# proroklab/graph-conv-memory

Hardware: AMD Instinct MI355X
Metric: belief-states/sec (BxT) DenseGCM fwd+bwd, graph_size=128 F=32 (higher is better)
Workload: dtype f32; 1 GPU; cfg2: DenseGCM + TemporalBackedge([1,2,4]), B=256/GPU, graph_size=128, obs=32, hidden=32, 2x DenseGraphConv+tanh, T=128; one bench step = one rollout through the per-step drop-in call surface `for t: mx, m = gcm(obs[t], m)` + backward; B_per_gpu=256, graph_size=128, obs=32, hidden=32, T=128, state=donated (DenseGCM(donate_state=True): hidden state advanced in place), parallelism=dp1 (batch-sharded, 1 flat-bucket all-reduce per backward)

## Files before the change

graph-conv-memory_amd/csrc/rows_cached_run.hip:

```cpp
#include <atomic>
#include <new>
#include <type_traits>

#include "fused_common.h"
#include "gcm_common.h"
#include "rows_common.h"
#include "rows_head.h"
#include "rows_lean.h"

namespace gcm_rows {

constexpr int RUN_CAP = GCM_ROWS_MAX_STEPS;
constexpr int RUN_WAVES = 8;
constexpr int RUN_PAIRS = RUN_CAP / 2 / RUN_WAVES;
constexpr int RUN_OCTS = RUN_CAP / 8 / RUN_WAVES;
constexpr int RUN_WSTAGE = 2 * 16 * 64 / (64 * RUN_WAVES);

struct RunTable {
  const float* obs[RUN_CAP];
  float* rec[RUN_CAP];
};

struct FreshArgs {
  HeadSrcs hs;
  float* packed;
  float* image;
  unsigned pad0, pad0_end, pad1, pad1_end;
};
struct NoFresh {};
constexpr int RUN_ADJ_TAB = 256 + 128;

#ifndef GCM_RUN_FRESH_STORES_LATE
#define GCM_RUN_FRESH_STORES_LATE 0
#endif

template <bool FRESH>
__global__ __launch_bounds__(64 * RUN_WAVES) void k_step_rows_cached_img4_lean_run(
    const float* __restrict__ image, float* __restrict__ nodes, float* __restrict__ cH, const float* __restrict__ params,
    int cur0_arg, int n, unsigned hops4, unsigned nhs, float* __restrict__ adj, int64_t* __restrict__ count,
    float* __restrict__ cA, float* __restrict__ cX, uint32_t* __restrict__ flags, unsigned o_v, unsigned o_hdr,
    unsigned o_coef, unsigned o_live, int rec, RunTable tab, std::conditional_t<FRESH, FreshArgs, NoFresh> fr) {
  constexpr int F = 32, H1 = 32, ROWS = 128 * 32;
  const int cur0 = FRESH ? 0 : cur0_arg;
  __shared__ __attribute__((aligned(16))) float sXH[2 * ROWS];
  __shared__ __attribute__((aligned(16))) float svw[RUN_WAVES * 128];
  __shared__ __attribute__((aligned(16))) f32x2 sW[2 * 16 * 32 * 2];
  __shared__ float sadj[FRESH ? RUN_ADJ_TAB : 1];
  const int lane = threadIdx.x & 63;
  const int wv = __builtin_amdgcn_readfirstlane((int)(threadIdx.x >> 6));
  const unsigned gb = blockIdx.x;
  const unsigned N = nhs & 0xffu;
  const int H2 = (int)((nhs >> 8) & 0xffu);
  const bool self = (nhs >> 16) & 1u;
  const unsigned g0 = gb * N;
  const int fl = lane & 31, hs = lane >> 5;
  float* sv = svw + 128 * wv + 64 * hs;
  const int ol = fl < H2 ? fl : H2 - 1;
  float* recd[RUN_OCTS];
#pragma unroll
  for (int j = 0; j < RUN_OCTS; ++j) {
    const int t = 8 * (wv + RUN_WAVES * j) + (lane >> 3);
    recd[j] = tab.rec[t < n ? t : n - 1];
  }
  float xo[RUN_PAIRS];
  float* recp[RUN_PAIRS];
#pragma unroll
  for (int j = 0; j < RUN_PAIRS; ++j) {
    const int t = 2 * (wv + RUN_WAVES * j) + hs;
    const int tc = t < n ? t : n - 1;
    xo[j] = tab.obs[tc][gb * F + fl];
    recp[j] = tab.rec[tc];
  }
  f32x2 wst[RUN_WSTAGE];
  f32x4 wq[2];
  float bias1, bias2;
  float v_img = 0.f, v_pack = 0.f;
  const size_t e_first = (size_t)gb + (size_t)gridDim.x * threadIdx.x, e_wave = (size_t)gb + (size_t)gridDim.x * (64 * wv);
  if constexpr (!FRESH) {
    const f32x2* i3 = reinterpret_cast<const f32x2*>(image + 2 * 4 * 64 * 64);
#pragma unroll
    for (int r = 0; r < RUN_WSTAGE; ++r) wst[r] = i3[(int)threadIdx.x + 64 * RUN_WAVES * r];
    const float* b1 = params + 2 * H1 * F;
    bias1 = b1[fl];
    bias2 = b1[H1 + 2 * H2 * H1 + ol];
  } else {
#pragma unroll
    for (int r = 0; r < 2; ++r) {
      const int q = (int)threadIdx.x + 64 * RUN_WAVES * r;
      const int m = q >> 8, h = (q >> 3) & 31;
      const float* w = m == 0 ? fr.hs.p[0] : m == 1 ? fr.hs.p[1] : m == 2 ? fr.hs.p[3] : fr.hs.p[4];
      wq[r] = f32x4{0.f, 0.f, 0.f, 0.f};
      if (m < 2 || h < H2) wq[r] = *reinterpret_cast<const f32x4*>(w + h * 32 + 4 * (q & 7));
    }
    bias1 = fr.hs.p[2][fl];
    bias2 = fr.hs.p[5][ol];
    if (e_wave < (size_t)IMG_LAYOUT_FLOATS && e_first < (size_t)IMG_LAYOUT_FLOATS) {
      const int e = (int)e_first;
      v_img = head_image_value(fr.hs, e >> 12, (e >> 6) & 63, e & 63, F, H1, H2);
    }
    if (e_wave < fr.hs.off[HEAD_MAX_SRCS] && e_first < fr.hs.off[HEAD_MAX_SRCS])
      v_pack = head_packed_value(fr.hs, (unsigned)e_first);
  }
  int hmax = 0, nh = 0;
#pragma unroll
  for (int i = 0; i < 4; ++i) {
    const int h = (int)((hops4 >> (8 * i)) & 0xffu);
    if (h != 0xff) {
      ++nh;
      if (h > hmax) hmax = h;
    }
  }
  {
    const int lo = cur0 - hmax > 0 ? cur0 - hmax : 0;
    const float* src = hs ? cH : nodes;
    for (int r = lo + wv; r < cur0; r += RUN_WAVES) sXH[hs * ROWS + r * 32 + fl] = src[(g0 + (unsigned)r) * 32 + fl];
  }
  if constexpr (!FRESH) {
#pragma unroll
    for (int r = 0; r < RUN_WSTAGE; ++r) {
      const int e = (int)threadIdx.x + 64 * RUN_WAVES * r;
      sW[image3_lds_pair(e)] = wst[r];
    }
  } else {
    float* sWf = reinterpret_cast<float*>(sW);
#pragma unroll
    for (int r = 0; r < 2; ++r) {
      const int q = (int)threadIdx.x + 64 * RUN_WAVES * r;
#pragma unroll
      for (int u = 0; u < 4; ++u) sWf[image3_lds_index(q >> 8, 4 * (q & 7) + u, (q >> 3) & 31)] = wq[r][u];
    }
    if (threadIdx.x < RUN_ADJ_TAB) {
      const int d = 128 - (int)threadIdx.x;
      bool hit = d == 0 && self;
#pragma unroll
      for (int i = 0; i < 4; ++i) hit = hit || (d > 0 && (int)((hops4 >> (8 * i)) & 0xffu) == d);
      sadj[threadIdx.x] = hit && threadIdx.x < 256 ? 1.f : 0.f;
    }
  }
#pragma unroll
  for (int j = 0; j < RUN_PAIRS; ++j) {
    const int t = 2 * (wv + RUN_WAVES * j) + hs;
    if (t < n) {
      sXH[(cur0 + t) * 32 + fl] = xo[j];
      const unsigned at = (g0 + (unsigned)(cur0 + t)) * F + fl;
      nodes[at] = xo[j];
      cX[at] = xo[j];
    }
  }
  __syncthreads();
  auto fresh_stores = [&]() {
    if constexpr (FRESH) {
      const f32x4 z = {0.f, 0.f, 0.f, 0.f};
      const int nq = (int)(N >> 2);
      f32x4* arow = reinterpret_cast<f32x4*>(adj + (size_t)g0 * N);
      for (int r = 2 * wv + hs; r < (int)N; r += 2 * RUN_WAVES) {
        if (fl < nq) {
          const float* at = sadj + (r < n ? 128 + 4 * fl - r : 256);
          arow[r * nq + fl] = f32x4{at[0], at[1], at[2], at[3]};
        }
      }
      f32x4* nrow = reinterpret_cast<f32x4*>(nodes + (size_t)g0 * F);
      for (int i = n * (F / 4) + (int)threadIdx.x; i < (int)N * (F / 4); i += 64 * RUN_WAVES) nrow[i] = z;
      if (gb == 0 && threadIdx.x < 64) {
        if (fr.pad0 + threadIdx.x < fr.pad0_end) nodes[fr.pad0 + threadIdx.x] = 0.f;
        if (fr.pad1 + threadIdx.x < fr.pad1_end) nodes[fr.pad1 + threadIdx.x] = 0.f;
      }
// ... 21 lines not shown
  for (int q = 0; q < 4; ++q) {
    const int idx = nh - 1 - q;
    has[q] = idx >= 0;
    back[q] = has[q] ? 32 * (int)((hops4 >> (8 * (idx & 3))) & 0xffu) : 0;
  }
  auto sources_all = [&](int cur, const float* rows, float (&va)[4]) {
    const float* at = rows + cur * 32 + fl;
#pragma unroll
    for (int q = 0; q < 4; ++q) {
      const float v = *(at - back[q]);
      va[q] = has[q] ? v : 0.f;
    }
  };
  f32x2 wa[16], wb[16];
  auto weights = [&](int layer) {
#pragma unroll
    for (int k = 0; k < 16; ++k) {
      const f32x4 q = *reinterpret_cast<const f32x4*>(sW + ((layer * 16 + k) * 32 + fl) * 2);
      wa[k] = f32x2{q[0], q[1]};
      wb[k] = f32x2{q[2], q[3]};
    }
  };
  auto matvec = [&]() { return lean_half_chain(wa, sv, 0) + lean_half_chain(wb, sv, 1); };
  weights(0);
  auto layer1 = [&](int cur, bool live, const float (&xa)[4]) {
    const unsigned rc = g0 + (unsigned)cur;
    const float xc = sXH[cur * 32 + fl];
    asm volatile("" ::: "memory");
    float agg1 = (xa[0] + xa[1]) + (xa[2] + xa[3]);
    agg1 = agg1 + (self ? xc : 0.f);
    *reinterpret_cast<f32x2*>(sv + 2 * fl) = f32x2{agg1, xc};
    asm volatile("" ::: "memory");
    const float p1 = bias1 + matvec();
    const float h1c = gcm_tanh(p1);
    asm volatile("" ::: "memory");
    if (live) {
      sXH[ROWS + cur * 32 + fl] = h1c;
      cA[rc * F + fl] = agg1;
      cH[rc * H1 + fl] = h1c;
    }
  };
#pragma unroll
  for (int j = 0; j < RUN_PAIRS; ++j) {
    const int t0 = 2 * (wv + RUN_WAVES * j);
    if (t0 >= n) break;
    const bool live = t0 + hs < n;
    const int cur = cur0 + (live ? t0 + hs : n - 1);
    float xa[4];
    if (cur0 + t0 < hmax) sources(cur, sXH, xa);
    else sources_all(cur, sXH, xa);
    layer1(cur, live, xa);
  }
  __syncthreads();
  weights(1);
  bool bad = false;
  auto layer2 = [&](int cur, bool live, float* saved, const float (&ha)[4]) {
    const float h1c = sXH[ROWS + cur * 32 + fl];
    asm volatile("" ::: "memory");
    float agg2 = (ha[0] + ha[1]) + (ha[2] + ha[3]);
    agg2 = agg2 + (self ? h1c : 0.f);
    *reinterpret_cast<f32x2*>(sv + 2 * fl) = f32x2{agg2, h1c};
    asm volatile("" ::: "memory");
    const float p2 = bias2 + matvec();
    const float v = gcm_tanh(p2);
    asm volatile("" ::: "memory");
    if (live && fl < H2) saved[gb * H2 + fl] = v;
    if (rec && live) {
      saved[o_v + gb * 2 * H1 + fl] = agg2;
      saved[o_v + gb * 2 * H1 + H1 + fl] = h1c;
    }
    bad = bad || (live && fl < H2 && !isfinite(v));
  };
#pragma unroll
  for (int j = 0; j < RUN_PAIRS; ++j) {
    const int t0 = 2 * (wv + RUN_WAVES * j);
    if (t0 >= n) break;
    const bool live = t0 + hs < n;
    const int cur = cur0 + (live ? t0 + hs : n - 1);
    float ha[4];
    if (cur0 + t0 < hmax) sources(cur, sXH + ROWS, ha);
    else sources_all(cur, sXH + ROWS, ha);
    layer2(cur, live, recp[j], ha);
  }
#pragma unroll
  for (int o = 0; o < RUN_OCTS; ++o) {
    const int t = 8 * (wv + RUN_WAVES * o) + (lane >> 3);
    if (t < n) {
      const int q = lane & 7;
      const int cur = cur0 + t;
      int k = 0;
#pragma unroll
      for (int i = 0; i < 4; ++i) k += (int)(((hops4 >> (8 * i)) & 0xffu) <= (unsigned)cur);
      const int j = q < k ? cur - (int)((hops4 >> (8 * ((k - 1 - q) & 3))) & 0xffu) : cur;
      const bool is_cur = q == k;
      if (!FRESH && (q < k || (is_cur && self))) adj[(size_t)(g0 + (unsigned)cur) * N + j] = 1.f;
      if (rec) {
        float* saved = recd[o];
        if (q <= k) {
          (reinterpret_cast<int*>(saved + o_live) + gb * N)[q] = j;
          (saved + o_coef + gb * N)[q] = (is_cur && !self) ? 0.f : 1.f;
        }
        if (q == 7) {
          int* hdr = reinterpret_cast<int*>(saved + o_hdr) + 4 * gb;
          hdr[0] = k + 1; hdr[1] = k; hdr[2] = cur; hdr[3] = 0;
        }
// ... 19 lines not shown
  int n = 0, cur0 = 0;
  float *nodes = nullptr, *adj = nullptr, *cH = nullptr, *cA = nullptr, *cX = nullptr;
  int64_t* count = nullptr;
  const float *params = nullptr, *image = nullptr;
  uint32_t* flags = nullptr;
  int B = 0, N = 0, H2 = 0, self = 0, rec = 0;
  unsigned hops4 = 0xffffffffu;
  RunTable tab;
  int cap = RUN_CAP;
  unsigned long long stat_cid = 0;
  int stat_nodes = 0, stat_merged = 0, stat_absorbed = 0;
  struct Head {
    hipGraphNode_t node = nullptr;
    unsigned long long cid = 0;
    hipStream_t stream = nullptr;
    HeadSrcs hs{};
    float *packed = nullptr, *image = nullptr;
    void* zero = nullptr;
    size_t zero_bytes = 0;
    int H2 = 0;
  } head;
  bool absorb = true, fresh = false;
  FreshArgs fr{};
};

static std::atomic<bool> g_merge_ok{true};
static std::atomic<int> g_route{0}, g_last_error{0};

static void merge_off(hipError_t e) {
  g_last_error = (int)e;
  g_merge_ok = false;
  (void)hipGetLastError();
}
static std::atomic<bool> g_absorb_ok{true};
static void absorb_off(hipError_t e) {
  g_last_error = (int)e;
  g_absorb_ok = false;
  (void)hipGetLastError();
}

struct RunArgs {
  int cur0, n, rec;
  unsigned hops4, nhs, o_v, o_hdr, o_coef, o_live;
  NoFresh none;
  void* ptr[20];
  hipKernelNodeParams p;
};
static void fill_args(Run& R, int n, RunArgs& a) {
  const CachedLayout lay = make_cached_layout(R.B, R.N, 32, R.H2);
  a.cur0 = R.cur0;
  a.n = n;
  a.rec = R.rec;
  a.hops4 = R.hops4;
  a.nhs = (unsigned)R.N | (unsigned)R.H2 << 8 | (R.self ? 1u << 16 : 0u);
  a.o_v = (unsigned)lay.o_v; a.o_hdr = (unsigned)lay.o_hdr; a.o_coef = (unsigned)lay.o_coef; a.o_live = (unsigned)lay.o_live;
  void* ptr[20] = {&R.image, &R.nodes, &R.cH, &R.params, &a.cur0, &a.n, &a.hops4, &a.nhs, &R.adj, &R.count,
                   &R.cA,    &R.cX,    &R.flags, &a.o_v, &a.o_hdr, &a.o_coef, &a.o_live, &a.rec, &R.tab,
                   R.fresh ? (void*)&R.fr : (void*)&a.none};
  for (int i = 0; i < 20; ++i) a.ptr[i] = ptr[i];
  a.p = hipKernelNodeParams{};
  a.p.func = R.fresh ? (void*)k_step_rows_cached_img4_lean_run<true> : (void*)k_step_rows_cached_img4_lean_run<false>;
  a.p.gridDim = dim3(R.B);
  a.p.blockDim = dim3(64 * RUN_WAVES);
  a.p.sharedMemBytes = 0;
  a.p.kernelParams = a.ptr;
  a.p.extra = nullptr;
}

inline int64_t pad64(int64_t v) { return (v + 63) & ~int64_t(63); }

static int absorb_head(Run& R, int n, hipGraph_t graph, hipError_t* broken) {
  const Run::Head& H = R.head;
  if (!R.absorb || !g_absorb_ok.load() || R.fresh || R.cur0 != 0 || !H.node || H.cid != R.cid || H.stream != R.stream)
    return 0;
  const int64_t n_nodes = pad64((int64_t)R.B * R.N * 32), n_adj = pad64((int64_t)R.B * R.N * R.N);
  const auto aligned16 = [](const void* p) { return (reinterpret_cast<uintptr_t>(p) & 15) == 0; };
  if (H.packed != R.params || H.image != R.image || H.H2 != R.H2 || R.N % 4 != 0 || H.zero != (void*)R.nodes ||
      H.zero_bytes != sizeof(float) * (size_t)(n_nodes + n_adj + 2 * (int64_t)R.B) || R.adj != R.nodes + n_nodes ||
      reinterpret_cast<float*>(R.count) != R.nodes + n_nodes + n_adj || !aligned16(H.hs.p[0]) || !aligned16(H.hs.p[1]) ||
      !aligned16(H.hs.p[3]) || !aligned16(H.hs.p[4]))
    return 0;
  size_t nd = 0, n_dep = 0, nh = 0;
  hipGraphNode_t one = nullptr, hdeps[8];
  hipError_t e = hipGraphNodeGetDependentNodes(R.node, nullptr, &n_dep);
// ... 267 lines not shown
  if (type != hipGraphNodeTypeKernel || got.func != lean_step_kernel()) return GCM_OK;
  R->node = node;
  R->cid = cid;
  R->stream = st;
  R->n = 1;
  R->cur0 = cur_host;
  R->nodes = nodes; R->adj = adj; R->count = count; R->cH = cache_h1; R->cA = cache_agg1; R->cX = cache_nodes;
  R->params = params; R->image = weight_image; R->flags = flags;
  R->B = B; R->N = N; R->H2 = H2; R->self = self; R->rec = record ? 1 : 0;
  R->hops4 = hops4;
  R->tab.obs[0] = obs;
  R->tab.rec[0] = saved;
  return GCM_OK;
}

extern "C" int gcm_rows_run_set_absorb(void* run, int on) {
  GCM_REQUIRE(run);
  static_cast<gcm_rows::Run*>(run)->absorb = on != 0;
  return GCM_OK;
}
extern "C" int gcm_rows_run_absorbed(const void* run) {
  return run ? static_cast<const gcm_rows::Run*>(run)->stat_absorbed : 0;
}
extern "C" int gcm_rows_run_absorb_enabled(void) { return gcm_rows::g_absorb_ok.load() ? 1 : 0; }

extern "C" int gcm_dense_rows_head_fused_run(void* run, const float* const* srcs_host, const size_t* lens_host, int n,
                                             float* packed, float* image, int F, int H1, int H2, void* zero,
                                             size_t zero_bytes, gcm_stream_t stream) {
  using namespace gcm_rows;
  const int rc = gcm_dense_rows_head_fused(srcs_host, lens_host, n, packed, image, F, H1, H2, zero, zero_bytes, stream);
  Run* R = static_cast<Run*>(run);
  if (!R) return rc;
  R->head.node = nullptr;
  if (rc != GCM_OK || !R->absorb || !g_absorb_ok.load() || !g_merge_ok.load() || !image || !zero || F != 32 || H1 != 32)
    return rc;
  hipStream_t st = (hipStream_t)stream;
  hipStreamCaptureStatus cs = hipStreamCaptureStatusNone;
  unsigned long long cid = 0;
  hipGraph_t graph = nullptr;
  const hipGraphNode_t* deps = nullptr;
  size_t nd = 0;
  hipError_t e = hipStreamGetCaptureInfo_v2(st, &cs, &cid, &graph, &deps, &nd);
  if (e != hipSuccess) {
    absorb_off(e);
    return rc;
  }
// ... 37 lines not shown
```

graph-conv-memory_amd/csrc/torch_ext/step_ext.cpp:

```cpp
#include <cstdlib>
#include <torch/extension.h>
#include <c10/hip/HIPFunctions.h>
#include <c10/hip/HIPStream.h>
#include <c10/hip/HIPGraphsC10Utils.h>
#include <torch/csrc/autograd/python_variable.h>

#include <algorithm>
#include <cstring>
#include <vector>

#include "gcm_hip.h"

#ifdef GCM_HOST_PROF
#include <chrono>
static double g_prof[8];
static long g_prof_n;
static inline double prof_now() {
  return std::chrono::duration<double, std::micro>(std::chrono::steady_clock::now().time_since_epoch()).count();
}
#define PROF_T(i) { const double t_ = prof_now(); g_prof[i] += t_ - prof_t; prof_t = t_; }
#else
#define PROF_T(i)
#endif

namespace {

using torch::autograd::AutogradContext;
using torch::autograd::variable_list;

inline int64_t pad64(int64_t n) { return (n + 63) & ~int64_t(63); }

struct StepCfg {
  std::vector<gcm_selector_desc> descs;
  int act1, act2, has_bias, N, F, H1, H2;
  int cached_flags = 0;
  bool col_cache = true;
  bool hops_bptt = true;
  bool hops_fold = true;
  bool merge_captured = true;
  int merge_cap = 0;
  bool absorb_head = true;
  int64_t P;
  bool has_distance = false;
  at::Tensor ws;
  size_t ws_bytes = 0;

  StepCfg(int64_t desc_ptr, int n_desc, int act1_, int act2_, int has_bias_, int N_, int F_,
          int H1_, int H2_)
      : act1(act1_), act2(act2_), has_bias(has_bias_), N(N_), F(F_), H1(H1_), H2(H2_) {
    descs.resize(n_desc);
    if (n_desc) std::memcpy(descs.data(), reinterpret_cast<const void*>(desc_ptr),
                            sizeof(gcm_selector_desc) * n_desc);
    for (const auto& d : descs) has_distance |= d.kind == GCM_SEL_DISTANCE;
    P = (int64_t)gcm_dense_gnn2_param_count(F, H1, H2);
  }

  void update_descs(int64_t desc_ptr, int n_desc) {
    if (n_desc == (int)descs.size() && n_desc)
      std::memcpy(descs.data(), reinterpret_cast<const void*>(desc_ptr),
                  sizeof(gcm_selector_desc) * n_desc);
  }

  void* workspace(int B, const at::Tensor& like, size_t* bytes) {
    *bytes = 0;
// ... 518 lines not shown
  std::shared_ptr<DxChain> dxc;
  std::shared_ptr<DxGateNode> dx_gate;
  std::shared_ptr<DxStepNode> dx_last;
  std::shared_ptr<RowsChainNode> node;
  std::vector<pybind11::object> hook_dicts;
  std::vector<pybind11::object> dicts, keys;
  std::vector<pybind11::object> objs;
  std::vector<uint32_t> vers;
  at::Tensor l_nodes, l_adj, l_weights, l_count;
  uint32_t lv_nodes = 0, lv_adj = 0, lv_count = 0;
  int64_t xB = -1, xF = -1, n_steps = 0;

  void note_versions() {
    lv_nodes = l_nodes._version();
    lv_adj = l_adj._version();
    lv_count = l_count._version();
  }
  bool state_untouched() const {
    return l_nodes.defined() && l_nodes._version() == lv_nodes && l_adj._version() == lv_adj &&
           l_count._version() == lv_count;
  }
  int dev = -1;
  void* mrun = nullptr;
  int mrun_cap = 0, mrun_absorb = -1;

  RowsFast(const std::vector<std::pair<pybind11::object, pybind11::object>>& specs,
           const std::vector<pybind11::object>& hooks)
      : hook_dicts(hooks) {
    for (const auto& s : specs) {
      dicts.push_back(s.first);
      keys.push_back(s.second);
    }
  }
  RowsFast(const RowsFast&) = delete;
  RowsFast& operator=(const RowsFast&) = delete;
  ~RowsFast() {
    if (mrun) gcm_rows_run_destroy(mrun);
  }
  bool last_cached_eager = true;
  void* merge_run() {
    last_cached_eager = rec_pool.capturing == 0;
    if (!cfg->merge_captured || rec_pool.capturing == 0) return nullptr;
    if (!mrun) mrun = gcm_rows_run_create();
    const int cap = cfg->merge_cap > 0 ? std::min(cfg->merge_cap, gcm_rows_run_steps_cap()) : gcm_rows_run_steps_cap();
    if (mrun && cap != mrun_cap) {
      gcm_rows_run_set_cap(mrun, cap);
      mrun_cap = cap;
    }
    set_absorb(cfg->absorb_head);
    return mrun;
  }
  void set_absorb(bool on) {
    if (mrun && (int)on != mrun_absorb) {
      gcm_rows_run_set_absorb(mrun, on ? 1 : 0);
      mrun_absorb = (int)on;
    }
  }
  void* head_run(bool on) {
    if (!on) {
      set_absorb(false);
      return nullptr;
    }
    if (!mrun) mrun = gcm_rows_run_create();
    set_absorb(true);
    return mrun;
  }
  std::pair<int, int> merge_stats() const {
    int out[2] = {0, 0};
    if (mrun && !last_cached_eager) gcm_rows_run_stats(mrun, out);
    return {out[0], out[1]};
  }
  int head_absorbed() const { return mrun && !last_cached_eager ? gcm_rows_run_absorbed(mrun) : 0; }

  bool hooks_registered() const {
    for (const auto& d : hook_dicts)
      if (PyObject_Size(d.ptr()) != 0) return true;
    return false;
  }

  bool params_current() const {
    for (size_t i = 0; i < dicts.size(); ++i) {
      PyObject* o = PyDict_GetItem(dicts[i].ptr(), keys[i].ptr());
      if (o != objs[i].ptr()) return false;
      if (o && THPVariable_Check(o) && THPVariable_Unpack(o)._version() != vers[i]) return false;
    }
    return true;
  }

  static bool want_donate(bool donate_, int dx_, const at::Tensor& head_nodes) {
    return donate_ && (dx_ == 0 || (dx_ == 1 && !(head_nodes.defined() && head_nodes.requires_grad())));
  }
  void arm(const at::Tensor& packed_, const at::Tensor& flags_, int64_t cfg_handle, bool donate_, int dx_ = 0,
           const at::Tensor& head_nodes = at::Tensor(), const at::Tensor& head_count = at::Tensor(),
           bool fresh = false) {
// ... 1937 lines not shown
    if (!same) {
      memo.taus = at::Tensor();
      TORCH_CHECK(false, "SparseGCM: `taus` was modified in place without moving its version counter (through .data?) "
                         "between two calls: the sizes of this call's tensors were taken from the call before");
    }
  }
  return (int64_t)(uint32_t)pinned.data_ptr<int32_t>()[0];
}

}

PYBIND11_MODULE(TORCH_EXTENSION_NAME, m) {
  m.doc() = "C++ autograd node of the fused DenseGCM step (host side of libgcm_hip.so)";
  pybind11::class_<StepCfg>(m, "StepCfg")
      .def(pybind11::init<int64_t, int, int, int, int, int, int, int, int>())
      .def("handle", [](StepCfg& c) { return reinterpret_cast<int64_t>(&c); })
      .def("update_descs", &StepCfg::update_descs)
      .def("set_cached_flags", [](StepCfg& c, int f) { c.cached_flags = f; })
      .def("set_hops_bptt", [](StepCfg& c, bool on) { c.hops_bptt = on; })
      .def("set_hops_fold", [](StepCfg& c, bool on) { c.hops_fold = on; })
      .def("set_col_cache", [](StepCfg& c, bool on) { c.col_cache = on; })
      .def("set_merge_captured", [](StepCfg& c, bool on, int cap) { c.merge_captured = on; c.merge_cap = cap; })
      .def("set_absorb_head", [](StepCfg& c, bool on) { c.absorb_head = on; })
      .def("cached_launches", [](StepCfg& c, int B) {
        return gcm_dense_rows_cached_launches(c.descs.empty() ? nullptr : c.descs.data(), (int)c.descs.size(),
                                              c.has_bias | c.cached_flags, B, c.N, c.F, c.H1, c.H2);
      });
  m.def("fused_step", &fused_step);
  pybind11::class_<RowsFast>(m, "RowsFast")
      .def(pybind11::init<const std::vector<std::pair<pybind11::object, pybind11::object>>&,
                          const std::vector<pybind11::object>&>())
      .def("run", &RowsFast::run)
      .def("step", &RowsFast::step)
      .def("continues", &RowsFast::continues)
      .def("edited_dx_state", &RowsFast::edited_dx_state)
      .def("donates", [](RowsFast& f) { return f.donate; })
      .def("pending", &RowsFast::pending)
      .def("forget", &RowsFast::forget)
      .def("set_head_image", &RowsFast::set_head_image)
      .def("steps", [](RowsFast& f) { return f.n_steps; })
      .def("cached_steps", [](RowsFast& f) { return f.cached_steps - f.col_steps; })
      .def("rolled_steps", [](RowsFast& f) { return f.rolled_steps; })
      .def("col_steps", [](RowsFast& f) { return f.col_steps; })
      .def("merge_stats", &RowsFast::merge_stats)
      .def("head_absorbed", &RowsFast::head_absorbed)
      .def("has_chain", [](RowsFast& f) { return f.node != nullptr || f.dxc != nullptr; });
  pybind11::class_<LearnedCfg>(m, "LearnedCfg")
      .def(pybind11::init<int, int, int, int, int, int, int, double, double, double>())
      .def("handle", [](LearnedCfg& c) { return reinterpret_cast<int64_t>(&c); });
  pybind11::class_<LearnedChain>(m, "LearnedChain")
      .def(pybind11::init<int64_t, const at::Tensor&, bool>())
      .def("cached_steps", &LearnedChain::n_cached)
      .def("total_steps", [](LearnedChain& c) { return c.all_steps; })
      .def("steady_steps", [](LearnedChain& c) { return c.steady_steps; })
      .def("donates", [](LearnedChain& c) { return c.donate; })
      .def("executed", &LearnedChain::executed)
      .def("recording", &LearnedChain::recording)
      .def("steps", &LearnedChain::steps);
  m.def("learned_step2", &learned_step2);
  m.def("pack_params", &pack_params);
  m.def("pack_params_head", &pack_params_head, pybind11::arg("tensors"), pybind11::arg("F"), pybind11::arg("H1"),
        pybind11::arg("H2"), pybind11::arg("want_image"), pybind11::arg("B"), pybind11::arg("N"), pybind11::arg("feats"),
        pybind11::arg("fast") = pybind11::none(), pybind11::arg("absorb") = false);
  pybind11::class_<LearnedFast>(m, "LearnedFast")
      .def(pybind11::init<const std::vector<std::pair<pybind11::object, pybind11::object>>&,
                          const std::vector<pybind11::object>&, pybind11::object>())
      .def("arm", &LearnedFast::arm)
      .def("step", &LearnedFast::step)
// ... 24 lines not shown
```

graph-conv-memory_amd/gcm/_hip.py:

```python
import ctypes
import os

import torch

from . import _abi

_LIB_PATH = os.path.join(os.path.dirname(os.path.abspath(__file__)), "_lib", "libgcm_hip.so")
_lib = None

_HEADER = _abi.header("gcm_hip.h")
PROTOTYPES = _abi.prototypes(_HEADER)
_CONSTANTS = _abi.constants(_HEADER)
_AGGR_HEADER = _abi.header("gcm_hip_aggr.h")
AGGR_PROTOTYPES = _abi.prototypes(_AGGR_HEADER)
_CONSTANTS.update(_abi.constants(_AGGR_HEADER))
_LEARNED_DET_HEADER = _abi.header("gcm_hip_learned_det.h")
LEARNED_DET_PROTOTYPES = _abi.prototypes(_LEARNED_DET_HEADER)
_TRANSFORMER_HEADER = _abi.header("gcm_hip_transformer.h")
TRANSFORMER_PROTOTYPES = _abi.prototypes(_TRANSFORMER_HEADER)
_RESET_HEADER = _abi.header("gcm_hip_reset.h")
RESET_PROTOTYPES = _abi.prototypes(_RESET_HEADER)
GIN_PROTOTYPES = _abi.prototypes(_abi.header("gcm_hip_gin.h"))
BPTT_HOPS_PROTOTYPES = _abi.prototypes(_abi.header("gcm_hip_bptt_hops.h"))
BPTT_HOPS_UNFOLDED_PROTOTYPES = _abi.prototypes(_abi.header("gcm_hip_bptt_hops_unfolded.h"))
# ... 1 lines not shown
GATED_PROTOTYPES = _abi.prototypes(_abi.header("gcm_hip_gated.h"))
TAG_PROTOTYPES = _abi.prototypes(_abi.header("gcm_hip_tag.h"))
_PNA_HEADER = _abi.header("gcm_hip_pna.h")
PNA_PROTOTYPES = _abi.prototypes(_PNA_HEADER)
_CONSTANTS.update(_abi.constants(_PNA_HEADER))
RGCN_PROTOTYPES = _abi.prototypes(_abi.header("gcm_hip_rgcn.h"))
GEN_PROTOTYPES = _abi.prototypes(_abi.header("gcm_hip_gen.h"))
EDGECONV_PROTOTYPES = _abi.prototypes(_abi.header("gcm_hip_edgeconv.h"))
_MP_HEADER = _abi.header("gcm_hip_mp.h")
MP_PROTOTYPES = _abi.prototypes(_MP_HEADER)
_CONSTANTS.update(_abi.constants(_MP_HEADER))
_BRIDGE_HEADER = _abi.header("gcm_hip_bridge.h")
BRIDGE_PROTOTYPES = _abi.prototypes(_BRIDGE_HEADER)
_CONSTANTS.update(_abi.constants(_BRIDGE_HEADER))
_WINDOW_HEADER = _abi.header("gcm_hip_window.h")
WINDOW_PROTOTYPES = _abi.prototypes(_WINDOW_HEADER)
_CONSTANTS.update(_abi.constants(_WINDOW_HEADER))
_SEGMENT_HEADER = _abi.header("gcm_hip_segments.h")
SEGMENT_PROTOTYPES = _abi.prototypes(_SEGMENT_HEADER)
_CONSTANTS.update(_abi.constants(_SEGMENT_HEADER))
HEAD_PROTOTYPES = _abi.prototypes(_abi.header("gcm_hip_head.h"))
RUN_PROTOTYPES = _abi.prototypes(_abi.header("gcm_hip_run.h"))
RUN_HEAD_PROTOTYPES = _abi.prototypes(_abi.header("gcm_hip_run_head.h"))
_KNN_HEADER = _abi.header("gcm_hip_knn.h")
KNN_PROTOTYPES = _abi.prototypes(_KNN_HEADER)
_CONSTANTS.update(_abi.constants(_KNN_HEADER))
globals().update({name[4:]: value for name, value in _CONSTANTS.items()})
GCM_EUNSUPPORTED = _CONSTANTS["GCM_EUNSUPPORTED"]
DIR = {d: _CONSTANTS["GCM_DIR_" + d.upper()] for d in ("forward", "backward", "both")}


class SelectorDesc(ctypes.Structure):
    _fields_ = _abi.struct_fields(_HEADER, "gcm_selector_desc")


class HipLibraryError(RuntimeError):
    pass


def bind(handle, prototypes=PROTOTYPES, names=None):
    for name in prototypes if names is None else names:
        fn = getattr(handle, name)
        fn.restype, fn.argtypes = prototypes[name]
    return handle


# ... 9 lines not shown
        handle = bind(ctypes.CDLL(os.environ.get("GCM_HIP_LIB") or _LIB_PATH))
        bind(handle, AGGR_PROTOTYPES)
        bind(handle, LEARNED_DET_PROTOTYPES)
        bind(handle, TRANSFORMER_PROTOTYPES)
        bind(handle, RESET_PROTOTYPES)
        bind(handle, GIN_PROTOTYPES)
        bind(handle, BPTT_HOPS_PROTOTYPES)
        bind(handle, BPTT_HOPS_UNFOLDED_PROTOTYPES)
        bind(handle, RESGATED_PROTOTYPES)
        bind(handle, GATED_PROTOTYPES)
        bind(handle, TAG_PROTOTYPES)
        bind(handle, PNA_PROTOTYPES)
        bind(handle, RGCN_PROTOTYPES)
        bind(handle, GEN_PROTOTYPES)
        bind(handle, EDGECONV_PROTOTYPES)
        bind(handle, MP_PROTOTYPES)
        bind(handle, BRIDGE_PROTOTYPES)
        bind(handle, WINDOW_PROTOTYPES)
        bind(handle, SEGMENT_PROTOTYPES)
        bind(handle, HEAD_PROTOTYPES)
        bind(handle, KNN_PROTOTYPES)
        bind(handle, RUN_PROTOTYPES)
        bind(handle, RUN_HEAD_PROTOTYPES)
        got, want = handle.gcm_abi_version(), _CONSTANTS["GCM_ABI_VERSION"]
        if got != want:
            raise HipLibraryError(f"{_LIB_PATH} has ABI revision {got}, include/gcm_hip.h is at {want}: "
                                  "rebuild the library (`python __graft_entry__.py`)")
        _lib = handle
    return _lib


def check(rc, what):
    if rc != 0:
        msg = lib().gcm_status_string(rc).decode()
        raise RuntimeError(f"{what} failed: {msg} (code {rc})")


def ptr(t):
    return None if t is None else t.data_ptr()


def stream():
    return torch._C._cuda_getCurrentRawStream(torch.cuda.current_device())


def on_device(*tensors):
# ... 15 lines not shown
```

graph-conv-memory_amd/gcm/gcm.py:

```python
import math
import os
from typing import Tuple, Union

import weakref

import torch

from . import _hip, _ops


_DTYPES = (torch.float32, torch.float32, torch.float32, torch.float32, torch.int64, 1)


class SparseToDense(torch.nn.Module):

    def forward(self, x, edge_index, batch_idx, B, N, edge_weight=None):
        B, N = int(B), int(N)
        if x.dim() != 2 or edge_index.dim() != 2 or edge_index.shape[0] != 2:
            raise ValueError("SparseToDense takes x [M,F] and edge_index [2,E]")
        if edge_weight is not None and edge_weight.numel() != edge_index.shape[1]:
            raise ValueError("edge_weight must hold one value per edge")
        M, F = x.shape
        if not x.is_cuda or F == 0:
            return self._torch_forward(x, edge_index, batch_idx, B, N, edge_weight)
# ... 146 lines not shown
        self._cfg_last = None
        self._packed_cache = None
        self._flags = {}
        self._pending = []
        self._pinned_pool = []
        self._ctr = [0]
        self._fast = None
        self._learned_chain = None
        self.noise_pool_steps = 64
        self.learned_cached_steps = True
        self.learned_fast_path = True
        self.rows_cached_steps = True
        self.rows_col_cache = os.environ.get("GCM_COL_CACHE", "1") == "1"
        self.rows_one_launch_distance = True
        self.rows_weight_image_v4 = os.environ.get("GCM_IMG_V4", "1") == "1"
        self.rows_bookkeeping_wave = os.environ.get("GCM_ONE_WAVE", "0") != "1"
        self.rows_lean_step = os.environ.get("GCM_LEAN_STEP", "1") == "1"
        self.rows_hops_bptt = os.environ.get("GCM_BPTT_HOPS", "1") == "1"
        self.rows_hops_fold = os.environ.get("GCM_BPTT_HOPS_FOLD", "1") == "1"
        self.rows_fused_head = os.environ.get("GCM_FUSED_HEAD", "1") == "1"
        self.rows_merge_captured = os.environ.get("GCM_MERGE_CAPTURED", "1") == "1"
        self.rows_merge_cap = None
        self.rows_absorb_head = os.environ.get("GCM_ABSORB_HEAD", "1") == "1"
        self._head_ready = None
        self.rollout_time_parallel = True
        self.rows_dx = True

    def get_initial_hidden_state(self, x):
        assert x.dim() == 2
        B, feats = x.shape
        edges = torch.zeros(B, self.graph_size, self.graph_size, device=x.device)
        nodes = torch.zeros(B, self.graph_size, feats, device=x.device)
        if self.edge_weights:
            weights = torch.zeros(B, self.graph_size, self.graph_size, device=x.device)
        else:
            weights = torch.zeros(0, device=x.device)
        num_nodes = torch.zeros(B, dtype=torch.long, device=x.device)
        return nodes, edges, weights, num_nodes

    def _fresh_state(self, x):
        if not x.is_cuda or x.dim() != 2 or x.dtype != torch.float32 or self.edge_weights:
            return self.get_initial_hidden_state(x)
        B, feats = x.shape
        N = self.graph_size
        pad = lambda n: (n + 63) & ~63
        n_nodes, n_adj = pad(B * N * feats), pad(B * N * N)
        flat = torch.zeros(n_nodes + n_adj + 2 * B, device=x.device)
        st = flat.untyped_storage()
        nodes = torch.empty(0, device=x.device).set_(st, 0, (B, N, feats))
        edges = torch.empty(0, device=x.device).set_(st, n_nodes, (B, N, N))
        num_nodes = torch.empty(0, dtype=torch.long, device=x.device).set_(st, (n_nodes + n_adj) // 2, (B,))
        return nodes, edges, torch.zeros(0, device=x.device), num_nodes

    def rows_steps(self):
        n = 0
        for cfg in self._cfg_cache.values():
            if cfg is not False and cfg._rows_fast is not None:
                n += cfg._rows_fast.steps()
        return n

    def merge_stats(self, head=False):
        nodes = merged = absorbed = 0
        for cfg in self._cfg_cache.values():
            if cfg is not False and cfg._rows_fast is not None:
                a, b = cfg._rows_fast.merge_stats()
                nodes, merged = nodes + a, merged + b
                absorbed += cfg._rows_fast.head_absorbed()
        out = {"nodes": nodes, "merged_steps": merged}
        if head:
            out["head_absorbed"] = absorbed
        return out

    def learned_fast_steps(self):
        n = 0
        for cfg in self._cfg_cache.values():
            if cfg is not False and cfg._learned_fast is not None:
                n += cfg._learned_fast.steps()
        return n

    def learned_steady_steps_taken(self):
        lc = self._learned_chain
        return int(lc[1].steady_steps()) if lc is not None else 0

    def rows_cached_steps_taken(self):
        n = 0
        for cfg in self._cfg_cache.values():
            if cfg is not False and cfg._rows_fast is not None:
                n += cfg._rows_fast.cached_steps()
        return n

    def rows_col_steps_taken(self):
        n = 0
        for cfg in self._cfg_cache.values():
# ... 397 lines not shown
            return self._forward_fused(x, nodes, adj, weights, num_nodes, cfg, flags, link)
        cont = fast.continues(nodes, adj, weights, num_nodes)
        root = self._packed_params(cfg, head=link is None and not cont)
        if not x.is_contiguous():
            x = x.contiguous()
        if not (nodes.is_contiguous() and adj.is_contiguous() and num_nodes.is_contiguous()):
            if self.donate_state:
                raise ValueError("donate_state=True needs contiguous hidden-state tensors")
            nodes, adj, num_nodes = nodes.contiguous(), adj.contiguous(), num_nodes.contiguous()
        fresh = getattr(nodes, "_gcm_fresh", False)
        if fresh:
            nodes._gcm_fresh = False
            if cfg.cpp_handle():
                cfg._cpp.set_cached_flags(
                    (0 if (self.rows_one_launch_distance or not cfg.has_distance) else _hip.STEP_TWO_LAUNCH)
                    | (_hip.STEP_IMG_V4 if self.rows_weight_image_v4 else 0)
                    | (0 if self.rows_bookkeeping_wave else _hip.STEP_ONE_WAVE)
                    | (0 if self.rows_lean_step else _hip.STEP_NOT_LEAN))
                cfg._cpp.set_col_cache(bool(self.rows_col_cache))
                cfg._cpp.set_hops_bptt(bool(self.rows_hops_bptt))
                cfg._cpp.set_hops_fold(bool(self.rows_hops_fold))
                cfg._cpp.set_merge_captured(bool(self.rows_merge_captured), int(self.rows_merge_cap or 0))
                cfg._cpp.set_absorb_head(bool(self.rows_absorb_head))
            image = self._packed_cache[5]
            if image is not None and self._packed_cache[1] is root:
                fast.set_head_image(root, image)
        mx, n2, a2, c2, donate = fast.run(x, nodes, adj, weights, num_nodes, root, flags, cfg.cpp_handle(),
                                          self.donate_state, need_dx, bool(fresh and self.rows_cached_steps))
        if donate:
            out = hidden
        else:
            if self.mutate_num_nodes_on_overflow:
                num_nodes.copy_(c2 - 1)
            out = (n2, a2, weights, c2)
        if self.mutate_num_nodes_on_overflow or cfg.sharded:
            self._fast = None
        else:
            every = {"deferred": self.poll_interval, "sync": 1, "off": float("inf")}[self.finite_check]
            self._fast = (fast.step, flags, every)
        if self.finite_check != "off":
            self._poll(flags)
        return mx, out

    def _forward_learned(self, x, hidden, cfg, flags, link):
        nodes, adj, weights, num_nodes = hidden
        root = self._packed_params(cfg, head=link is None)
# ... 370 lines not shown
```

include/gcm_hip.h:

```cpp
#ifndef GCM_HIP_H
#define GCM_HIP_H

#include <stddef.h>
#include <stdint.h>

#ifdef __cplusplus
extern "C" {
#endif

typedef void* gcm_stream_t;

#define GCM_OK 0
#define GCM_EINVAL (-1)
#define GCM_EUNSUPPORTED (-2)
#define GCM_EWORKSPACE (-3)

#define GCM_ACT_NONE 0
#define GCM_ACT_TANH 1
#define GCM_ACT_RELU 2

#define GCM_DIR_FORWARD 1
#define GCM_DIR_BACKWARD 2
#define GCM_DIR_BOTH 3

// ... 404 lines not shown

int gcm_dense_rows_cached_supported(const gcm_selector_desc* selectors, int n_selectors, int has_bias, int N,
                                    int F, int H1, int H2);
int gcm_dense_rows_cached_layout(int B, int N, int F, int H1, int H2, size_t* out5);
size_t gcm_dense_rows_cached_weight_image_floats(void);
int gcm_dense_rows_cached_weight_image(const float* params, float* image, int F, int H1, int H2,
                                       gcm_stream_t stream);
#include "gcm_hip_head.h"
int gcm_dense_rows_step_cached(const float* obs, float* nodes, float* adj, int64_t* count,
                               const gcm_selector_desc* selectors, int n_selectors, const float* params,
                               const float* weight_image, int has_bias, int act1, int act2, float* cache_h1, float* cache_agg1,
                               float* cache_nodes, float* saved, int record, int cur_host, uint32_t* flags, int B,
                               int N, int F, int H1, int H2, gcm_stream_t stream);
int gcm_dense_rows_cached_supported_ws(const gcm_selector_desc* selectors, int n_selectors, int has_bias, int N,
                                       int F, int H1, int H2);
int gcm_dense_rows_step_cached_ws(const float* obs, float* nodes, float* adj, int64_t* count,
                                  const gcm_selector_desc* selectors, int n_selectors, const float* params,
                                  const float* weight_image, int has_bias, int act1, int act2, float* cache_h1,
                                  float* cache_agg1, float* cache_nodes, float* saved, int record, int cur_host,
                                  uint32_t* flags, void* workspace, size_t workspace_bytes, int B, int N, int F,
                                  int H1, int H2, gcm_stream_t stream);
#include "gcm_hip_run.h"
#include "gcm_hip_run_head.h"
int gcm_dense_rows_cached_roll_supported(const gcm_selector_desc* selectors, int n_selectors, int has_bias, int N,
                                         int F, int H1, int H2);
int gcm_dense_rows_step_cached_roll(const float* obs, float* nodes, const gcm_selector_desc* selectors, int n_selectors,
                                    const float* params, const float* weight_image, int has_bias, int act1, int act2,
                                    float* cache_h1, float* cache_agg1, float* cache_nodes, float* saved, int record,
                                    int t_abs, uint32_t* flags, int B, int N, int F, int H1, int H2,
                                    gcm_stream_t stream);
int gcm_dense_rows_colcache_supported(const gcm_selector_desc* selectors, int n_selectors, int has_bias, int N,
                                      int F, int H1, int H2);
int gcm_dense_rows_step_colcache_functional(const float* obs, const float* nodes_in, const float* adj_in,
                                            const int64_t* count_in, float* nodes_out, float* adj_out,
                                            int64_t* count_out, const gcm_selector_desc* selectors, int n_selectors,
                                            const float* params, int has_bias, int act1, int act2, float* cache_agg1,
                                            float* cache_root, float* saved, int record, int cur_host, uint32_t* flags,
                                            int B, int N, int F, int H1, int H2, gcm_stream_t stream);
int gcm_dense_rows_step_colcache(const float* obs, float* nodes, float* adj, int64_t* count,
                                 const gcm_selector_desc* selectors, int n_selectors, const float* params,
                                 int has_bias, int act1, int act2, float* cache_agg1, float* cache_root, float* saved,
                                 int record, int cur_host, uint32_t* flags, int B, int N, int F, int H1, int H2,
                                 gcm_stream_t stream);
int gcm_edge_distance_step_cached_supported(int n_cur_rows, int B, int N, int F, int H1, int H2);
int gcm_dense_rows_cached_launches(const gcm_selector_desc* selectors, int n_selectors, int has_bias, int B, int N,
                                   int F, int H1, int H2);
// ... 216 lines not shown
```

Measured before the change: 554.3 million belief-states/s.

## Compute run kernel GraphConv layers with MFMA 16x16x4 f32 tiles

Adds an MFMA variant of the fused multi-step run kernel. Each wave now processes 16 timesteps as a matrix tile and computes both DenseGraphConv layers with f32 MFMA instructions instead of per-lane LDS matvec chains. The LDS row stride is padded (default 36) to reduce bank conflicts on the new tile operand loads. It is enabled by default through a config flag, env var and C API toggle, and it adds compile-time cut macros for profiling. The cost is that each step's partial products are summed in a different order, and each wave needs many accumulator registers.

```diff
diff --git a/graph-conv-memory_amd/csrc/rows_cached_run.hip b/graph-conv-memory_amd/csrc/rows_cached_run.hip
--- a/graph-conv-memory_amd/csrc/rows_cached_run.hip
+++ b/graph-conv-memory_amd/csrc/rows_cached_run.hip
@@ -34,16 +34,26 @@
 #define GCM_RUN_FRESH_STORES_LATE 0
 #endif
 
-template <bool FRESH>
+#ifndef GCM_RUN_CUT
+#define GCM_RUN_CUT 0
+#endif
+#ifndef GCM_RUN_MFMA_CUT
+#define GCM_RUN_MFMA_CUT 0
+#endif
+#ifndef GCM_RUN_MFMA_RS
+#define GCM_RUN_MFMA_RS 36
+#endif
+
+template <bool FRESH, bool MFMA>
 __global__ __launch_bounds__(64 * RUN_WAVES) void k_step_rows_cached_img4_lean_run(
     const float* __restrict__ image, float* __restrict__ nodes, float* __restrict__ cH, const float* __restrict__ params,
     int cur0_arg, int n, unsigned hops4, unsigned nhs, float* __restrict__ adj, int64_t* __restrict__ count,
     float* __restrict__ cA, float* __restrict__ cX, uint32_t* __restrict__ flags, unsigned o_v, unsigned o_hdr,
     unsigned o_coef, unsigned o_live, int rec, RunTable tab, std::conditional_t<FRESH, FreshArgs, NoFresh> fr) {
-  constexpr int F = 32, H1 = 32, ROWS = 128 * 32;
+  constexpr int F = 32, H1 = 32, RS = MFMA ? GCM_RUN_MFMA_RS : 32, ROWS = 128 * RS;
   const int cur0 = FRESH ? 0 : cur0_arg;
   __shared__ __attribute__((aligned(16))) float sXH[2 * ROWS];
-  __shared__ __attribute__((aligned(16))) float svw[RUN_WAVES * 128];
+  __shared__ __attribute__((aligned(16))) float svw[MFMA ? 4 : RUN_WAVES * 128];
   __shared__ __attribute__((aligned(16))) f32x2 sW[2 * 16 * 32 * 2];
   __shared__ float sadj[FRESH ? RUN_ADJ_TAB : 1];
   const int lane = threadIdx.x & 63;
@@ -74,6 +84,19 @@
   f32x2 wst[RUN_WSTAGE];
   f32x4 wq[2];
   float bias1, bias2;
+  const int ar = lane & 15, ak = lane >> 4;
+  float* rec_a = nullptr;
+  float* rec_c[4] = {nullptr, nullptr, nullptr, nullptr};
+  float b1c[2] = {0.f, 0.f}, b2c[2] = {0.f, 0.f};
+  if constexpr (MFMA) {
+    const int ta = 16 * wv + ar;
+    rec_a = tab.rec[ta < n ? ta : n - 1];
+#pragma unroll
+    for (int v = 0; v < 4; ++v) {
+      const int tc = 16 * wv + 4 * ak + v;
+      rec_c[v] = tab.rec[tc < n ? tc : n - 1];
+    }
+  }
   float v_img = 0.f, v_pack = 0.f;
   const size_t e_first = (size_t)gb + (size_t)gridDim.x * threadIdx.x, e_wave = (size_t)gb + (size_t)gridDim.x * (64 * wv);
   if constexpr (!FRESH) {
@@ -83,6 +106,14 @@
     const float* b1 = params + 2 * H1 * F;
     bias1 = b1[fl];
     bias2 = b1[H1 + 2 * H2 * H1 + ol];
+    if constexpr (MFMA) {
+#pragma unroll
+      for (int ct = 0; ct < 2; ++ct) {
+        const int col = 16 * ct + ar;
+        b1c[ct] = b1[col];
+        b2c[ct] = b1[H1 + 2 * H2 * H1 + (col < H2 ? col : H2 - 1)];
+      }
+    }
   } else {
 #pragma unroll
     for (int r = 0; r < 2; ++r) {
@@ -94,6 +125,14 @@
     }
     bias1 = fr.hs.p[2][fl];
     bias2 = fr.hs.p[5][ol];
+    if constexpr (MFMA) {
+#pragma unroll
+      for (int ct = 0; ct < 2; ++ct) {
+        const int col = 16 * ct + ar;
+        b1c[ct] = fr.hs.p[2][col];
+        b2c[ct] = fr.hs.p[5][col < H2 ? col : H2 - 1];
+      }
+    }
     if (e_wave < (size_t)IMG_LAYOUT_FLOATS && e_first < (size_t)IMG_LAYOUT_FLOATS) {
       const int e = (int)e_first;
       v_img = head_image_value(fr.hs, e >> 12, (e >> 6) & 63, e & 63, F, H1, H2);
@@ -113,7 +152,7 @@
   {
     const int lo = cur0 - hmax > 0 ? cur0 - hmax : 0;
     const float* src = hs ? cH : nodes;
-    for (int r = lo + wv; r < cur0; r += RUN_WAVES) sXH[hs * ROWS + r * 32 + fl] = src[(g0 + (unsigned)r) * 32 + fl];
+    for (int r = lo + wv; r < cur0; r += RUN_WAVES) sXH[hs * ROWS + r * RS + fl] = src[(g0 + (unsigned)r) * 32 + fl];
   }
   if constexpr (!FRESH) {
 #pragma unroll
@@ -141,7 +180,7 @@
   for (int j = 0; j < RUN_PAIRS; ++j) {
     const int t = 2 * (wv + RUN_WAVES * j) + hs;
     if (t < n) {
-      sXH[(cur0 + t) * 32 + fl] = xo[j];
+      sXH[(cur0 + t) * RS + fl] = xo[j];
       const unsigned at = (g0 + (unsigned)(cur0 + t)) * F + fl;
       nodes[at] = xo[j];
       cX[at] = xo[j];
@@ -209,7 +248,106 @@
     }
   };
   auto matvec = [&]() { return lean_half_chain(wa, sv, 0) + lean_half_chain(wb, sv, 1); };
-  weights(0);
+  const bool act = 16 * wv < n;
+  const bool live_a = 16 * wv + ar < n;
+  const int cur_a = cur0 + (live_a ? 16 * wv + ar : n - 1);
+  int so[4];
+  bool sa[4];
+  {
+    int k = 0;
+#pragma unroll
+    for (int i = 0; i < 4; ++i) k += (int)(((hops4 >> (8 * i)) & 0xffu) <= (unsigned)cur_a);
+#pragma unroll
+    for (int q = 0; q < 4; ++q) {
+      const int idx = k - 1 - q;
+      sa[q] = idx >= 0;
+      so[q] = sa[q] ? RS * (cur_a - (int)((hops4 >> (8 * (idx & 3))) & 0xffu)) : 0;
+    }
+  }
+  auto operands = [&](const float* rows, f32x2 (&ag)[4], f32x2 (&own)[4]) {
+    const float* at = rows + 2 * ak;
+#pragma unroll
+    for (int qf = 0; qf < 4; ++qf) {
+      own[qf] = *reinterpret_cast<const f32x2*>(at + cur_a * RS + 8 * qf);
+      f32x2 v[4];
+#pragma unroll
+      for (int q = 0; q < 4; ++q) {
+        const f32x2 u = *reinterpret_cast<const f32x2*>(at + so[q] + 8 * qf);
+        v[q] = sa[q] ? u : f32x2{0.f, 0.f};
+      }
+      ag[qf] = (v[0] + v[1]) + (v[2] + v[3]);
+      ag[qf] = ag[qf] + (self ? own[qf] : f32x2{0.f, 0.f});
+    }
+  };
+  f32x4 acc[2][2][2][2];
+  auto products = [&](int layer, const f32x2 (&ag)[4], const f32x2 (&own)[4]) {
+    const float* sWf = reinterpret_cast<const float*>(sW);
+    f32x4 bw[2][2][2];
+#pragma unroll
+    for (int i = 0; i < 2; ++i)
+#pragma unroll
+      for (int p = 0; p < 2; ++p)
+#pragma unroll
+        for (int ct = 0; ct < 2; ++ct)
+          bw[i][p][ct] = *reinterpret_cast<const f32x4*>(sWf + ((layer * 16 + 8 * i + 2 * ak + p) * 32 + 16 * ct + ar) * 4);
+#pragma unroll
+    for (int ct = 0; ct < 2; ++ct)
+#pragma unroll
+      for (int kh = 0; kh < 2; ++kh)
+#pragma unroll
+        for (int p = 0; p < 2; ++p)
+#pragma unroll
+          for (int m = 0; m < 2; ++m) acc[ct][kh][p][m] = f32x4{0.f, 0.f, 0.f, 0.f};
+    if (GCM_RUN_MFMA_CUT & 1) {
+#pragma unroll
+      for (int ct = 0; ct < 2; ++ct) acc[ct][0][0][0] = f32x4{ag[0][0] + bw[0][0][ct][0], own[1][1] + bw[1][1][ct][1], ag[2][0], own[3][1]};
+      return;
+    }
+#pragma unroll
+    for (int i = 0; i < 2; ++i)
+#pragma unroll
+      for (int kh = 0; kh < 2; ++kh)
+#pragma unroll
+        for (int p = 0; p < 2; ++p)
+#pragma unroll
+          for (int ct = 0; ct < 2; ++ct) {
+            const int qf = 2 * kh + i;
+            acc[ct][kh][p][0] = __builtin_amdgcn_mfma_f32_16x16x4f32(ag[qf][p], bw[i][p][ct][2 * kh], acc[ct][kh][p][0], 0, 0, 0);
+            acc[ct][kh][p][1] = __builtin_amdgcn_mfma_f32_16x16x4f32(own[qf][p], bw[i][p][ct][2 * kh + 1], acc[ct][kh][p][1], 0, 0, 0);
+          }
+  };
+  auto tree = [&](int ct, int v) {
+    const float s0 = (acc[ct][0][0][0][v] + acc[ct][0][1][0][v]) + (acc[ct][0][0][1][v] + acc[ct][0][1][1][v]);
+    const float s1 = (acc[ct][1][0][0][v] + acc[ct][1][1][0][v]) + (acc[ct][1][0][1][v] + acc[ct][1][1][1][v]);
+    return s0 + s1;
+  };
+  auto run_tanh = [](float v) { return (GCM_RUN_MFMA_CUT & 2) ? v : gcm_tanh(v); };
+  constexpr bool STORES = !(GCM_RUN_MFMA_CUT & 4);
+  bool bad = false;
+  if constexpr (MFMA) {
+    if (act) {
+      f32x2 ag[4], own[4];
+      operands(sXH, ag, own);
+      if (STORES && live_a) {
+        float* to = cA + (size_t)(g0 + (unsigned)cur_a) * F + 2 * ak;
+#pragma unroll
+        for (int qf = 0; qf < 4; ++qf) *reinterpret_cast<f32x2*>(to + 8 * qf) = ag[qf];
+      }
+      products(0, ag, own);
+#pragma unroll
+      for (int ct = 0; ct < 2; ++ct)
+#pragma unroll
+        for (int v = 0; v < 4; ++v) {
+          const int t = 16 * wv + 4 * ak + v;
+          const float h1c = run_tanh(b1c[ct] + tree(ct, v));
+          if (t < n) {
+            sXH[ROWS + (cur0 + t) * RS + 16 * ct + ar] = h1c;
+            if (STORES) cH[(size_t)(g0 + (unsigned)(cur0 + t)) * H1 + 16 * ct + ar] = h1c;
+          }
+        }
+    }
+  }
+  if constexpr (!MFMA) weights(0);
   auto layer1 = [&](int cur, bool live, const float (&xa)[4]) {
     const unsigned rc = g0 + (unsigned)cur;
     const float xc = sXH[cur * 32 + fl];
@@ -227,20 +365,45 @@
       cH[rc * H1 + fl] = h1c;
     }
   };
-#pragma unroll
-  for (int j = 0; j < RUN_PAIRS; ++j) {
-    const int t0 = 2 * (wv + RUN_WAVES * j);
-    if (t0 >= n) break;
-    const bool live = t0 + hs < n;
-    const int cur = cur0 + (live ? t0 + hs : n - 1);
-    float xa[4];
-    if (cur0 + t0 < hmax) sources(cur, sXH, xa);
-    else sources_all(cur, sXH, xa);
-    layer1(cur, live, xa);
+  if constexpr (!MFMA && GCM_RUN_CUT < 2) {
+#pragma unroll
+    for (int j = 0; j < RUN_PAIRS; ++j) {
+      const int t0 = 2 * (wv + RUN_WAVES * j);
+      if (t0 >= n) break;
+      const bool live = t0 + hs < n;
+      const int cur = cur0 + (live ? t0 + hs : n - 1);
+      float xa[4];
+      if (cur0 + t0 < hmax) sources(cur, sXH, xa);
+      else sources_all(cur, sXH, xa);
+      layer1(cur, live, xa);
+    }
   }
   __syncthreads();
-  weights(1);
-  bool bad = false;
+  if constexpr (MFMA) {
+    if (act) {
+      f32x2 ag[4], own[4];
+      operands(sXH + ROWS, ag, own);
+      if (STORES && rec && live_a) {
+        float* to = rec_a + o_v + gb * 2 * H1 + 2 * ak;
+#pragma unroll
+        for (int qf = 0; qf < 4; ++qf) {
+          *reinterpret_cast<f32x2*>(to + 8 * qf) = ag[qf];
+          *reinterpret_cast<f32x2*>(to + H1 + 8 * qf) = own[qf];
+        }
+      }
+      products(1, ag, own);
+#pragma unroll
+      for (int ct = 0; ct < 2; ++ct)
+#pragma unroll
+        for (int v = 0; v < 4; ++v) {
+          const bool out = 16 * wv + 4 * ak + v < n && 16 * ct + ar < H2;
+          const float mx = run_tanh(b2c[ct] + tree(ct, v));
+          if (STORES && out) rec_c[v][gb * H2 + 16 * ct + ar] = mx;
+          bad = bad || (out && !isfinite(mx));
+        }
+    }
+  }
+  if constexpr (!MFMA) weights(1);
   auto layer2 = [&](int cur, bool live, float* saved, const float (&ha)[4]) {
     const float h1c = sXH[ROWS + cur * 32 + fl];
     asm volatile("" ::: "memory");
@@ -258,16 +421,18 @@
     }
     bad = bad || (live && fl < H2 && !isfinite(v));
   };
-#pragma unroll
-  for (int j = 0; j < RUN_PAIRS; ++j) {
-    const int t0 = 2 * (wv + RUN_WAVES * j);
-    if (t0 >= n) break;
-    const bool live = t0 + hs < n;
-    const int cur = cur0 + (live ? t0 + hs : n - 1);
-    float ha[4];
-    if (cur0 + t0 < hmax) sources(cur, sXH + ROWS, ha);
-    else sources_all(cur, sXH + ROWS, ha);
-    layer2(cur, live, recp[j], ha);
+  if constexpr (!MFMA && GCM_RUN_CUT < 1) {
+#pragma unroll
+    for (int j = 0; j < RUN_PAIRS; ++j) {
+      const int t0 = 2 * (wv + RUN_WAVES * j);
+      if (t0 >= n) break;
+      const bool live = t0 + hs < n;
+      const int cur = cur0 + (live ? t0 + hs : n - 1);
+      float ha[4];
+      if (cur0 + t0 < hmax) sources(cur, sXH + ROWS, ha);
+      else sources_all(cur, sXH + ROWS, ha);
+      layer2(cur, live, recp[j], ha);
+    }
   }
 #pragma unroll
   for (int o = 0; o < RUN_OCTS; ++o) {
@@ -333,6 +498,7 @@
   } head;
   bool absorb = true, fresh = false;
   FreshArgs fr{};
+  bool mfma = true;
 };
 
 static std::atomic<bool> g_merge_ok{true};
@@ -370,7 +536,8 @@
                    R.fresh ? (void*)&R.fr : (void*)&a.none};
   for (int i = 0; i < 20; ++i) a.ptr[i] = ptr[i];
   a.p = hipKernelNodeParams{};
-  a.p.func = R.fresh ? (void*)k_step_rows_cached_img4_lean_run<true> : (void*)k_step_rows_cached_img4_lean_run<false>;
+  a.p.func = R.fresh ? (R.mfma ? (void*)k_step_rows_cached_img4_lean_run<true, true> : (void*)k_step_rows_cached_img4_lean_run<true, false>)
+                     : (R.mfma ? (void*)k_step_rows_cached_img4_lean_run<false, true> : (void*)k_step_rows_cached_img4_lean_run<false, false>);
   a.p.gridDim = dim3(R.B);
   a.p.blockDim = dim3(64 * RUN_WAVES);
   a.p.sharedMemBytes = 0;
@@ -684,6 +851,12 @@
 extern "C" int gcm_rows_run_absorbed(const void* run) {
   return run ? static_cast<const gcm_rows::Run*>(run)->stat_absorbed : 0;
 }
+extern "C" int gcm_rows_run_set_mfma(void* run, int on) {
+  GCM_REQUIRE(run);
+  static_cast<gcm_rows::Run*>(run)->mfma = on != 0;
+  return GCM_OK;
+}
+extern "C" int gcm_rows_run_mfma(const void* run) { return run && static_cast<const gcm_rows::Run*>(run)->mfma ? 1 : 0; }
 extern "C" int gcm_rows_run_absorb_enabled(void) { return gcm_rows::g_absorb_ok.load() ? 1 : 0; }
 
 extern "C" int gcm_dense_rows_head_fused_run(void* run, const float* const* srcs_host, const size_t* lens_host, int n,
diff --git a/graph-conv-memory_amd/csrc/torch_ext/step_ext.cpp b/graph-conv-memory_amd/csrc/torch_ext/step_ext.cpp
--- a/graph-conv-memory_amd/csrc/torch_ext/step_ext.cpp
+++ b/graph-conv-memory_amd/csrc/torch_ext/step_ext.cpp
@@ -40,6 +40,7 @@
   bool merge_captured = true;
   int merge_cap = 0;
   bool absorb_head = true;
+  bool run_mfma = true;
   int64_t P;
   bool has_distance = false;
   at::Tensor ws;
@@ -604,7 +605,7 @@
   }
   int dev = -1;
   void* mrun = nullptr;
-  int mrun_cap = 0, mrun_absorb = -1;
+  int mrun_cap = 0, mrun_absorb = -1, mrun_mfma = -1;
 
   RowsFast(const std::vector<std::pair<pybind11::object, pybind11::object>>& specs,
            const std::vector<pybind11::object>& hooks)
@@ -630,6 +631,10 @@
       mrun_cap = cap;
     }
     set_absorb(cfg->absorb_head);
+    if (mrun && (int)cfg->run_mfma != mrun_mfma) {
+      gcm_rows_run_set_mfma(mrun, cfg->run_mfma ? 1 : 0);
+      mrun_mfma = (int)cfg->run_mfma;
+    }
     return mrun;
   }
   void set_absorb(bool on) {
@@ -652,6 +657,7 @@
     if (mrun && !last_cached_eager) gcm_rows_run_stats(mrun, out);
     return {out[0], out[1]};
   }
+  bool run_mfma() const { return mrun ? gcm_rows_run_mfma(mrun) != 0 : (cfg ? cfg->run_mfma : true); }
   int head_absorbed() const { return mrun && !last_cached_eager ? gcm_rows_run_absorbed(mrun) : 0; }
 
   bool hooks_registered() const {
@@ -2635,6 +2641,7 @@
       .def("set_col_cache", [](StepCfg& c, bool on) { c.col_cache = on; })
       .def("set_merge_captured", [](StepCfg& c, bool on, int cap) { c.merge_captured = on; c.merge_cap = cap; })
       .def("set_absorb_head", [](StepCfg& c, bool on) { c.absorb_head = on; })
+      .def("set_run_mfma", [](StepCfg& c, bool on) { c.run_mfma = on; })
       .def("cached_launches", [](StepCfg& c, int B) {
         return gcm_dense_rows_cached_launches(c.descs.empty() ? nullptr : c.descs.data(), (int)c.descs.size(),
                                               c.has_bias | c.cached_flags, B, c.N, c.F, c.H1, c.H2);
@@ -2657,6 +2664,7 @@
       .def("col_steps", [](RowsFast& f) { return f.col_steps; })
       .def("merge_stats", &RowsFast::merge_stats)
       .def("head_absorbed", &RowsFast::head_absorbed)
+      .def("run_mfma", &RowsFast::run_mfma)
       .def("has_chain", [](RowsFast& f) { return f.node != nullptr || f.dxc != nullptr; });
   pybind11::class_<LearnedCfg>(m, "LearnedCfg")
       .def(pybind11::init<int, int, int, int, int, int, int, double, double, double>())
diff --git a/graph-conv-memory_amd/gcm/_hip.py b/graph-conv-memory_amd/gcm/_hip.py
--- a/graph-conv-memory_amd/gcm/_hip.py
+++ b/graph-conv-memory_amd/gcm/_hip.py
@@ -47,6 +47,7 @@
 HEAD_PROTOTYPES = _abi.prototypes(_abi.header("gcm_hip_head.h"))
 RUN_PROTOTYPES = _abi.prototypes(_abi.header("gcm_hip_run.h"))
 RUN_HEAD_PROTOTYPES = _abi.prototypes(_abi.header("gcm_hip_run_head.h"))
+RUN_MFMA_PROTOTYPES = _abi.prototypes(_abi.header("gcm_hip_run_mfma.h"))
 _KNN_HEADER = _abi.header("gcm_hip_knn.h")
 KNN_PROTOTYPES = _abi.prototypes(_KNN_HEADER)
 _CONSTANTS.update(_abi.constants(_KNN_HEADER))
@@ -102,6 +103,7 @@
         bind(handle, KNN_PROTOTYPES)
         bind(handle, RUN_PROTOTYPES)
         bind(handle, RUN_HEAD_PROTOTYPES)
+        bind(handle, RUN_MFMA_PROTOTYPES)
         got, want = handle.gcm_abi_version(), _CONSTANTS["GCM_ABI_VERSION"]
         if got != want:
             raise HipLibraryError(f"{_LIB_PATH} has ABI revision {got}, include/gcm_hip.h is at {want}: "
diff --git a/graph-conv-memory_amd/gcm/gcm.py b/graph-conv-memory_amd/gcm/gcm.py
--- a/graph-conv-memory_amd/gcm/gcm.py
+++ b/graph-conv-memory_amd/gcm/gcm.py
@@ -192,6 +192,7 @@
         self.rows_merge_captured = os.environ.get("GCM_MERGE_CAPTURED", "1") == "1"
         self.rows_merge_cap = None
         self.rows_absorb_head = os.environ.get("GCM_ABSORB_HEAD", "1") == "1"
+        self.rows_run_mfma = os.environ.get("GCM_RUN_MFMA", "1") == "1"
         self._head_ready = None
         self.rollout_time_parallel = True
         self.rows_dx = True
@@ -229,16 +230,20 @@
                 n += cfg._rows_fast.steps()
         return n
 
-    def merge_stats(self, head=False):
+    def merge_stats(self, head=False, form=False):
         nodes = merged = absorbed = 0
+        mfma = bool(self.rows_run_mfma)
         for cfg in self._cfg_cache.values():
             if cfg is not False and cfg._rows_fast is not None:
                 a, b = cfg._rows_fast.merge_stats()
                 nodes, merged = nodes + a, merged + b
                 absorbed += cfg._rows_fast.head_absorbed()
+                mfma = mfma and bool(cfg._rows_fast.run_mfma())
         out = {"nodes": nodes, "merged_steps": merged}
         if head:
             out["head_absorbed"] = absorbed
+        if form:
+            out["run_mfma"] = mfma
         return out
 
     def learned_fast_steps(self):
@@ -682,6 +687,7 @@
                 cfg._cpp.set_hops_fold(bool(self.rows_hops_fold))
                 cfg._cpp.set_merge_captured(bool(self.rows_merge_captured), int(self.rows_merge_cap or 0))
                 cfg._cpp.set_absorb_head(bool(self.rows_absorb_head))
+                cfg._cpp.set_run_mfma(bool(self.rows_run_mfma))
             image = self._packed_cache[5]
             if image is not None and self._packed_cache[1] is root:
                 fast.set_head_image(root, image)
diff --git a/include/gcm_hip.h b/include/gcm_hip.h
--- a/include/gcm_hip.h
+++ b/include/gcm_hip.h
@@ -450,6 +450,7 @@
                                   int H1, int H2, gcm_stream_t stream);
 #include "gcm_hip_run.h"
 #include "gcm_hip_run_head.h"
+#include "gcm_hip_run_mfma.h"
 int gcm_dense_rows_cached_roll_supported(const gcm_selector_desc* selectors, int n_selectors, int has_bias, int N,
                                          int F, int H1, int H2);
 int gcm_dense_rows_step_cached_roll(const float* obs, float* nodes, const gcm_selector_desc* selectors, int n_selectors,
diff --git a/include/gcm_hip_run_mfma.h b/include/gcm_hip_run_mfma.h
--- /dev/null
+++ b/include/gcm_hip_run_mfma.h
@@ -0,0 +1,7 @@
+#ifndef GCM_HIP_RUN_MFMA_H
+#define GCM_HIP_RUN_MFMA_H
+
+int gcm_rows_run_set_mfma(void* run, int on);
+int gcm_rows_run_mfma(const void* run);
+
+#endif
```

Result: faster. 582.6 million belief-states/s (median of 6 runs) (+5.1%).
